# yanqinJiang/Animate3D

Measured on NVIDIA H100. Metric: MV-VDM denoise-steps/sec @ 4view x 16frame x 256^2, higher is better.
Workload: dtype fp16

## Files before the change

### animate3d_b200/csrc/a3d_gemm.cu

```cuda
#include <type_traits>

#include "a3d_common.cuh"
#include "a3d_host.cuh"
#include "a3d_wgmma.cuh"

namespace a3d {

struct GemmDev {
  int64_t M, N, K;
  int num_k_blocks;
  int tiles_m, tiles_n;
  int a_mode;
  int cpb;
  int conv_s;
  int tpi;
  int boh;
  int bimg;
  int tpr;
  int conv_pad;
  const float* bias;
  const float* rowbias;
  int64_t rb_ld, rb_div, rb_mod;
  float acc_scale;
  const __half* R1; int64_t ldr1; float r1_scale;
  const __half* R2; int64_t ldr2;
  void* C; int64_t ldc;
  int geglu, out_f32;
  int64_t perm_a, perm_b;
  long long* trace;
};

__device__ __forceinline__ float gelu_erf(float x) {
  float t;
  asm("rcp.approx.ftz.f32 %0, %1;" : "=f"(t) : "f"(fmaf(0.3275911f * 0.70710678118654752f, fabsf(x), 1.0f)));
  float poly = fmaf(1.061405429f, t, -1.453152027f);
  poly = fmaf(poly, t, 1.421413741f);
  poly = fmaf(poly, t, -0.284496736f);
  poly = fmaf(poly, t, 0.254829592f);
  const float xs = x * 0.84932180028801904f;
  const float e = ex2_approx(-xs * xs);
  const float erf_abs = fmaf(-(poly * t), e, 1.0f);
  const float h = 0.5f * x;
  return fmaf(fabsf(h), erf_abs, h);
}

__device__ __forceinline__ int64_t perm_row(int64_t m, int64_t a, int64_t b) {
  if (a == 0) return m;
  const int64_t ab = a * b;
  return (m / ab) * ab + (m % b) * a + (m / b) % a;
}

constexpr int kBM = 128;
constexpr int kBK = 64;
constexpr int kGemmThreads = 288;

template <int BN>
struct GemmCfg {
  static constexpr int kABytes = kBM * kBK * 2;
  static constexpr int kBBytes = BN * kBK * 2;
  static constexpr int kStageBytes = kABytes + kBBytes;
  static constexpr int kStages = (227 * 1024 - 1024 - 256) / kStageBytes > 6 ? 6 : (227 * 1024 - 1024 - 256) / kStageBytes;
  static constexpr int kSmemBytes = kStages * kStageBytes + 1024  + 256 ;
  static_assert(kSmemBytes <= 227 * 1024, "shared memory budget");
};

template <int BN>
__device__ __forceinline__ void wgmma_tile(float (&d)[BN / 2], uint64_t adesc, uint64_t bdesc, uint32_t acc) {
  if constexpr (BN == 256) wgmma_ss_n256<0>(d, adesc, bdesc, acc);
  else if constexpr (BN == 160) wgmma_ss_n160<0>(d, adesc, bdesc, acc);
  else wgmma_ss_n128<0>(d, adesc, bdesc, acc);
}

enum { kEpiPlain = 0, kEpiRes = 1, kEpiGeglu = 2, kEpiF32 = 3 };

template <int BN, int EPI>
struct EpiChunk {
  static constexpr int G = BN == 256 ? 1 + (EPI == kEpiGeglu) : 2;
  static constexpr bool kAhead = BN != 256;
  float bias[G][2];
  float rb[2][G][2];
  uint32_t r1[2][G], r2[2][G];
};

template <int EPI, int G>
__device__ __forceinline__ constexpr int epi_group(int c, int s) {
  if constexpr (EPI != kEpiGeglu) {
    return c * G + s;
  } else {
    const int o = c * (G / 2) + s % (G / 2);
    return (o / 4) * 8 + o % 4 + (s >= G / 2 ? 4 : 0);
  }
}

__device__ __forceinline__ void prefetch_l2(const void* a) { asm volatile("prefetch.global.L2 [%0];" ::"l"(a)); }

template <int BN, int EPI>
__global__ void __launch_bounds__(kGemmThreads, 1)
gemm_tc_kernel(const GemmDev p, const __grid_constant__ CUtensorMap mapA, const __grid_constant__ CUtensorMap mapB) {
  static_assert(EPI != kEpiGeglu || BN % 64 == 0, "GEGLU pairs a value with its gate inside 64-column blocks");
  static_assert((BN / 8) % EpiChunk<BN, EPI>::G == 0, "the tile's column groups split into whole chunks");
  using Cfg = GemmCfg<BN>;
  constexpr int kStages = Cfg::kStages;
  extern __shared__ uint8_t smem_raw[];
  uint8_t* smem = reinterpret_cast<uint8_t*>((reinterpret_cast<uintptr_t>(smem_raw) + 1023) & ~uintptr_t(1023));
  uint8_t* smem_a = smem;
  uint8_t* smem_b = smem + kStages * Cfg::kABytes;
  uint64_t* full_bar = reinterpret_cast<uint64_t*>(smem + kStages * Cfg::kStageBytes);
  uint64_t* empty_bar = full_bar + kStages;

  const int warp = threadIdx.x >> 5;
  const int lane = threadIdx.x & 31;
  const int num_tiles = p.tiles_m * p.tiles_n;

  if (warp == 8 && lane == 0) {
    tma_prefetch_desc(&mapA);
    tma_prefetch_desc(&mapB);
    for (int i = 0; i < kStages; ++i) {
      mbar_init(&full_bar[i], 1);
      mbar_init(&empty_bar[i], 8);
    }
    mbar_fence_init();
  }
  __syncthreads();

  if (warp == 8) {
    if (lane == 0) {
      int stage = 0;
      uint32_t phase = 0;
      for (int tile = blockIdx.x; tile < num_tiles; tile += gridDim.x) {
        const int mt = tile / p.tiles_n, nt = tile % p.tiles_n;
        int img0 = 0, oh0 = 0, ow0 = 0;
        if (p.a_mode == A3D_A_CONV3) {
          if (p.tpr > 1) { img0 = mt / p.tpi; oh0 = (mt % p.tpi) / p.tpr; ow0 = ((mt % p.tpi) % p.tpr) * kBM; }
          else if (p.tpi > 0) { img0 = mt / p.tpi; oh0 = (mt % p.tpi) * p.boh; }
          else { img0 = mt * p.bimg; oh0 = 0; }
        }
        for (int kb = 0; kb < p.num_k_blocks; ++kb) {
          mbar_wait(&empty_bar[stage], phase ^ 1);
          mbar_expect_tx(&full_bar[stage], Cfg::kStageBytes);
          if (p.a_mode == A3D_A_CONV3) {
            const int tap = kb / p.cpb, c0 = (kb % p.cpb) * kBK;
            const int ky = tap / 3, kx = tap % 3;
            tma_load_5d(smem_a + stage * Cfg::kABytes, &mapA, &full_bar[stage], c0, ow0 * p.conv_s + kx - p.conv_pad,
                        oh0 * p.conv_s + ky - p.conv_pad, img0, 0);
          } else {
            tma_load_5d(smem_a + stage * Cfg::kABytes, &mapA, &full_bar[stage], kb * kBK, mt * kBM, 0, 0, 0);
          }
          tma_load_5d(smem_b + stage * Cfg::kBBytes, &mapB, &full_bar[stage], kb * kBK, nt * BN, 0, 0, 0);
          if (++stage == kStages) { stage = 0; phase ^= 1; }
        }
      }
    }
    return;
  }

  const int wg = warp >> 2;
  const int g = lane >> 2, t = lane & 3;
  int stage = 0;
  uint32_t phase = 0;
  int tcount = 0;
  float acc[BN / 2];
  for (int tile = blockIdx.x; tile < num_tiles; tile += gridDim.x, ++tcount) {
    const int mt = tile / p.tiles_n, nt = tile % p.tiles_n;
    const bool tr = p.trace && blockIdx.x == 0 && threadIdx.x == 0 && tcount < 60;
    if (tr) p.trace[tcount * 16 + 0] = clock64();
    const int64_t col_base = (int64_t)nt * BN + 2 * t;
    int64_t row[2], orow[2];
#pragma unroll
    for (int h = 0; h < 2; ++h) {
      row[h] = (int64_t)mt * kBM + wg * 64 + (warp & 3) * 16 + g + 8 * h;
      orow[h] = (EPI == kEpiRes) ? perm_row(row[h], p.perm_a, p.perm_b) : row[h];
    }
    int prev_stage = -1;
    for (int kb = 0; kb < p.num_k_blocks; ++kb) {
      if constexpr (EPI == kEpiRes) {
        if (kb == (p.num_k_blocks > 2 ? p.num_k_blocks - 2 : 0)) {
          const int64_t ncols = p.N - (int64_t)nt * BN < BN ? p.N - (int64_t)nt * BN : BN;
          auto fetch = [&](const __half* a, bool ok) {
            const uintptr_t e = reinterpret_cast<uintptr_t>(a + ncols), l0 = reinterpret_cast<uintptr_t>(a) & ~uintptr_t(127);
#pragma unroll
            for (int i = 0; i < (2 * BN / 128 + 4) / 4; ++i) {
              const uintptr_t l = l0 + 128 * (t + 4 * i);
              if (ok && l < e) prefetch_l2(reinterpret_cast<const void*>(l));
            }
          };
#pragma unroll
          for (int h = 0; h < 2; ++h) {
            fetch(p.R1 + row[h] * p.ldr1 + (int64_t)nt * BN, p.R1 && row[h] < p.M);
            fetch(p.R2 + orow[h] * p.ldr2 + (int64_t)nt * BN, p.R2 && row[h] < p.M);
          }
        }
      }
      mbar_wait(&full_bar[stage], phase);
      const uint32_t a0 = smem_u32(smem_a + stage * Cfg::kABytes + wg * (64 * 128));
      const uint32_t b0 = smem_u32(smem_b + stage * Cfg::kBBytes);
      wgmma_fence();
#pragma unroll
      for (int k = 0; k < kBK / 16; ++k)
        wgmma_tile<BN>(acc, make_smem_desc_sw128(a0 + 32 * k, 16, 1024), make_smem_desc_sw128(b0 + 32 * k, 16, 1024),
                       (kb | k) ? 1u : 0u);
      wgmma_commit();
      wgmma_wait<1>();
      if (prev_stage >= 0 && lane == 0) mbar_arrive(&empty_bar[prev_stage]);
      prev_stage = stage;
      if (++stage == kStages) { stage = 0; phase ^= 1; }
    }

    using Chunk = EpiChunk<BN, EPI>;
    constexpr int G = Chunk::G;
    constexpr int kChunks = BN / 8 / G;
    const float* rb[2];
#pragma unroll
    for (int h = 0; h < 2; ++h) rb[h] = p.rowbias ? p.rowbias + ((row[h] / p.rb_div) % p.rb_mod) * p.rb_ld : nullptr;
    Chunk op;
    auto load_chunk = [&](int c) {
#pragma unroll
      for (int s = 0; s < G; ++s) {
        const int64_t n = col_base + 8 * epi_group<EPI, G>(c, s);
        const bool col_ok = n < p.N;
        op.bias[s][0] = (p.bias && col_ok) ? p.bias[n] : 0.f;
        op.bias[s][1] = (p.bias && col_ok) ? p.bias[n + 1] : 0.f;
#pragma unroll
        for (int h = 0; h < 2; ++h) {
          const bool ok = col_ok && row[h] < p.M;
          op.rb[h][s][0] = (rb[h] && ok) ? rb[h][n] : 0.f;
          op.rb[h][s][1] = (rb[h] && ok) ? rb[h][n + 1] : 0.f;
          if constexpr (EPI == kEpiRes) {
            op.r1[h][s] = (p.R1 && ok) ? *reinterpret_cast<const uint32_t*>(p.R1 + row[h] * p.ldr1 + n) : 0u;
            op.r2[h][s] = (p.R2 && ok) ? *reinterpret_cast<const uint32_t*>(p.R2 + orow[h] * p.ldr2 + n) : 0u;
          }
        }
      }
    };
    auto finish = [&](float v, int h, int s, int e) {
      if (p.bias) v += op.bias[s][e];
      if (rb[h]) v += op.rb[h][s][e];
      return v * p.acc_scale;
    };
    auto half2_float2 = [](uint32_t u) { return __half22float2(*reinterpret_cast<const __half2*>(&u)); };

    if constexpr (Chunk::kAhead) load_chunk(0);
    wgmma_wait<0>();
    reg_fence(acc);
    if (lane == 0) mbar_arrive(&empty_bar[prev_stage]);
    if (tr) p.trace[tcount * 16 + 1] = clock64();

#pragma unroll
    for (int c = 0; c < kChunks; ++c) {
      if constexpr (!Chunk::kAhead) load_chunk(c);
      if constexpr (EPI == kEpiGeglu) {
        uint32_t out[2][G / 2];
#pragma unroll
        for (int h = 0; h < 2; ++h)
#pragma unroll
          for (int s = 0; s < G / 2; ++s) {
            const int ju = epi_group<EPI, G>(c, s), jg = epi_group<EPI, G>(c, s + G / 2);
            const float u0 = finish(acc[4 * ju + 2 * h], h, s, 0), u1 = finish(acc[4 * ju + 2 * h + 1], h, s, 1);
            const float g0 = finish(acc[4 * jg + 2 * h], h, s + G / 2, 0), g1 = finish(acc[4 * jg + 2 * h + 1], h, s + G / 2, 1);
            out[h][s] = pack_f16x2(u0 * gelu_erf(g0), u1 * gelu_erf(g1));
          }
        if (Chunk::kAhead && c + 1 < kChunks) load_chunk(c + 1);
#pragma unroll
        for (int h = 0; h < 2; ++h) {
          if (row[h] >= p.M) continue;
          __half* crow = reinterpret_cast<__half*>(p.C) + row[h] * p.ldc;
#pragma unroll
          for (int s = 0; s < G / 2; ++s) {
            if (col_base + 8 * epi_group<EPI, G>(c, s) >= p.N) continue;
            const int o = c * (G / 2) + s;
            *reinterpret_cast<uint32_t*>(crow + (int64_t)nt * (BN / 2) + 8 * o + 2 * t) = out[h][s];
          }
        }
      } else if constexpr (EPI == kEpiF32) {
        float out[2][G][2];
#pragma unroll
        for (int h = 0; h < 2; ++h)
#pragma unroll
          for (int s = 0; s < G; ++s)
#pragma unroll
            for (int e = 0; e < 2; ++e) out[h][s][e] = finish(acc[4 * (c * G + s) + 2 * h + e], h, s, e);
        if (Chunk::kAhead && c + 1 < kChunks) load_chunk(c + 1);
#pragma unroll
        for (int h = 0; h < 2; ++h) {
          if (row[h] >= p.M) continue;
          float* crow = reinterpret_cast<float*>(p.C) + row[h] * p.ldc;
#pragma unroll
          for (int s = 0; s < G; ++s) {
            const int64_t n = col_base + 8 * (c * G + s);
            if (n >= p.N) continue;
            crow[n] = out[h][s][0];
            crow[n + 1] = out[h][s][1];
          }
        }
      } else {
        uint32_t out[2][G];
#pragma unroll
        for (int h = 0; h < 2; ++h)
#pragma unroll
          for (int s = 0; s < G; ++s) {
            const int j = c * G + s;
            float v0 = finish(acc[4 * j + 2 * h], h, s, 0), v1 = finish(acc[4 * j + 2 * h + 1], h, s, 1);
            if constexpr (EPI == kEpiRes) {
              if (p.R1) {
                const float2 f = half2_float2(op.r1[h][s]);
                v0 += p.r1_scale * f.x; v1 += p.r1_scale * f.y;
              }
              if (p.R2) {
                const float2 f = half2_float2(op.r2[h][s]);
                v0 += f.x; v1 += f.y;
              }
            }
            out[h][s] = pack_f16x2(v0, v1);
          }
        if (Chunk::kAhead && c + 1 < kChunks) load_chunk(c + 1);
#pragma unroll
        for (int h = 0; h < 2; ++h) {
          if (row[h] >= p.M) continue;
          __half* crow = reinterpret_cast<__half*>(p.C) + orow[h] * p.ldc;
#pragma unroll
          for (int s = 0; s < G; ++s) {
            const int64_t n = col_base + 8 * (c * G + s);
            if (n >= p.N) continue;
            *reinterpret_cast<uint32_t*>(crow + n) = out[h][s];
          }
        }
      }
    }
    if (tr) p.trace[tcount * 16 + 2] = clock64();
  }
}

struct SimtConv { int n, h, w, c, s, oh, ow, pad; };

__global__ void gemm_simt_kernel(const GemmDev p, const __half* __restrict__ A, int64_t lda, const __half* __restrict__ B,
                                 SimtConv cv) {
  const int64_t n_out = p.geglu ? p.N / 2 : p.N;
  const int64_t idx = (int64_t)blockIdx.x * blockDim.x + threadIdx.x;
  if (idx >= p.M * n_out) return;
  const int64_t m = idx / n_out;
  const int64_t j = idx % n_out;
  auto dot = [&](int64_t n) {
    float acc = 0.f;
    const __half* b = B + n * p.K;
    if (p.a_mode == A3D_A_PLAIN) {
      const __half* a = A + m * lda;
      for (int64_t k = 0; k < p.K; ++k) acc += __half2float(a[k]) * __half2float(b[k]);
    } else {
      const int img = (int)(m / (cv.oh * cv.ow));
      const int oy = (int)((m / cv.ow) % cv.oh), ox = (int)(m % cv.ow);
      for (int tap = 0; tap < 9; ++tap) {
        const int iy = oy * cv.s + tap / 3 - cv.pad, ix = ox * cv.s + tap % 3 - cv.pad;
        if (iy < 0 || iy >= cv.h || ix < 0 || ix >= cv.w) continue;
        const __half* a = A + (((int64_t)img * cv.h + iy) * cv.w + ix) * cv.c;
        const __half* bb = b + (int64_t)tap * cv.c;
        for (int c = 0; c < cv.c; ++c) acc += __half2float(a[c]) * __half2float(bb[c]);
      }
    }
    return acc;
  };
  const int64_t orow = perm_row(m, p.perm_a, p.perm_b);
  const float* rb = p.rowbias ? p.rowbias + ((m / p.rb_div) % p.rb_mod) * p.rb_ld : nullptr;
  auto finish = [&](int64_t n) {
    float v = dot(n);
    if (p.bias) v += p.bias[n];
    if (rb) v += rb[n];
    return v * p.acc_scale;
  };
  if (p.geglu) {
    const int64_t blk = j / 32, e = j % 32;
    const int64_t nu = blk * 64 + e, ng = nu + 32;
    const float u = finish(nu), g = finish(ng);
    reinterpret_cast<__half*>(p.C)[orow * p.ldc + j] = __float2half_rn(u * gelu_erf(g));
    return;
  }
  float v = finish(j);
  if (p.R1) v += p.r1_scale * __half2float(p.R1[m * p.ldr1 + j]);
  if (p.R2) v += __half2float(p.R2[orow * p.ldr2 + j]);
  if (p.out_f32) reinterpret_cast<float*>(p.C)[orow * p.ldc + j] = v;
  else reinterpret_cast<__half*>(p.C)[orow * p.ldc + j] = __float2half_rn(v);
}

template <int BN, int EPI>
static int launch_tc_epi(const GemmDev& dev, const CUtensorMap* mapA, const CUtensorMap* mapB, cudaStream_t st) {
  using Cfg = GemmCfg<BN>;
  static bool attr_set = false;
  if (!attr_set) {
    A3D_CUDA_CHECK(cudaFuncSetAttribute(gemm_tc_kernel<BN, EPI>, cudaFuncAttributeMaxDynamicSharedMemorySize, Cfg::kSmemBytes));
    attr_set = true;
  }
  const int tiles = dev.tiles_m * dev.tiles_n;
  const int grid = tiles < sm_count() ? tiles : sm_count();
  gemm_tc_kernel<BN, EPI><<<grid, kGemmThreads, Cfg::kSmemBytes, st>>>(dev, *mapA, *mapB);
  A3D_LAUNCH_CHECK();
  return A3D_OK;
}

template <int BN>
static int launch_tc(const GemmDev& dev, const CUtensorMap* mapA, const CUtensorMap* mapB, cudaStream_t st) {
  if (dev.out_f32) return launch_tc_epi<BN, kEpiF32>(dev, mapA, mapB, st);
  if (dev.geglu) {
    if constexpr (BN % 64 == 0) return launch_tc_epi<BN, kEpiGeglu>(dev, mapA, mapB, st);
    else return fail(A3D_EINVAL, "a3d_gemm: GEGLU needs a 128- or 256-column tile");
  }
  if (dev.R1 || dev.R2 || dev.perm_a) return launch_tc_epi<BN, kEpiRes>(dev, mapA, mapB, st);
  return launch_tc_epi<BN, kEpiPlain>(dev, mapA, mapB, st);
}

static long long* g_gemm_trace = nullptr;

}

extern "C" int a3d_debug_set_gemm_trace(void* device_buffer_1024_int64) {
  a3d::g_gemm_trace = reinterpret_cast<long long*>(device_buffer_1024_int64);
  return A3D_OK;
}

extern "C" int a3d_gemm(const a3d_gemm_args* a, void* stream) {
  using namespace a3d;
  cudaStream_t st = reinterpret_cast<cudaStream_t>(stream);
  if (!a || !a->A || !a->B || !a->C) return fail(A3D_EINVAL, "a3d_gemm: null operand");
  if (a->M <= 0 || a->N <= 0 || a->K <= 0) return fail(A3D_EINVAL, "a3d_gemm: empty problem M=%lld N=%lld K=%lld",
                                                        (long long)a->M, (long long)a->N, (long long)a->K);
  GemmDev d;
  memset(&d, 0, sizeof(d));
  d.M = a->M; d.N = a->N; d.K = a->K;
  d.a_mode = a->a_mode;
  d.bias = a->bias; d.rowbias = a->rowbias; d.rb_ld = a->rb_ld;
  d.rb_div = a->rb_div > 0 ? a->rb_div : 1; d.rb_mod = a->rb_mod > 0 ? a->rb_mod : (int64_t)1 << 40;
  d.acc_scale = a->acc_scale;
  d.R1 = reinterpret_cast<const __half*>(a->R1); d.ldr1 = a->ldr1; d.r1_scale = a->r1_scale;
  d.R2 = reinterpret_cast<const __half*>(a->R2); d.ldr2 = a->ldr2;
  d.C = a->C; d.ldc = a->ldc; d.geglu = a->geglu; d.out_f32 = a->out_f32;
  d.perm_a = a->perm_a; d.perm_b = a->perm_b;
  d.trace = g_gemm_trace;
  if (a->geglu && (a->out_f32 || a->R1 || a->R2 || a->perm_a || (a->N % 128)))
    return fail(A3D_EINVAL, "a3d_gemm: GEGLU epilogue takes bias / row-bias only, fp16 output, N %% 128 == 0");
  if (a->out_f32 && (a->R1 || a->R2 || a->perm_a))
    return fail(A3D_EINVAL, "a3d_gemm: fp32 output supports bias / row-bias only");

  SimtConv cv{0, 0, 0, 0, 1, 0, 0};
  if (a->a_mode == A3D_A_CONV3) {
    const int s = a->conv_stride;
    if (s != 1 && s != 2) return fail(A3D_EINVAL, "a3d_gemm: conv stride must be 1 or 2");
    if (a->conv_h % s || a->conv_w % s) return fail(A3D_EINVAL, "a3d_gemm: conv H/W must be multiples of the stride");
    cv = SimtConv{a->conv_n, a->conv_h, a->conv_w, a->conv_c, s, a->conv_h / s, a->conv_w / s, a->conv_nopad_lo ? 0 : 1};
    if (a->K != 9LL * a->conv_c || a->M != (int64_t)cv.n * cv.oh * cv.ow)
      return fail(A3D_EINVAL, "a3d_gemm: conv geometry does not match M/K");
    d.conv_s = s;
  } else if (a->a_mode != A3D_A_PLAIN) {
    return fail(A3D_EINVAL, "a3d_gemm: unknown a_mode %d", a->a_mode);
  }

  bool tc_ok = (a->K % kBK == 0) && (a->N % (a->geglu ? 16 : 8) == 0) && ((reinterpret_cast<uintptr_t>(a->A) & 15) == 0) &&
               ((reinterpret_cast<uintptr_t>(a->B) & 15) == 0) && (a->ldc % 16 == 0) &&
               ((reinterpret_cast<uintptr_t>(a->C) & 31) == 0);
  if (a->a_mode == A3D_A_PLAIN) tc_ok = tc_ok && (a->lda % 8 == 0) && a->lda >= a->K;
  int boh = 0, bimg = 1, tpi = 0, tpr = 1;
  if (a->a_mode == A3D_A_CONV3) {
    tc_ok = tc_ok && (cv.c % kBK == 0);
    const int opix = cv.oh * cv.ow;
    if (cv.ow > kBM) {
      tc_ok = tc_ok && (cv.ow % kBM == 0);
      boh = 1; tpr = cv.ow / kBM; tpi = cv.oh * tpr; bimg = 1;
    } else if (opix >= kBM) {
      tc_ok = tc_ok && (opix % kBM == 0) && (kBM % cv.ow == 0);
      boh = kBM / cv.ow; tpi = opix / kBM; bimg = 1;
    } else {
      tc_ok = tc_ok && (kBM % opix == 0);
      boh = cv.oh; tpi = 0; bimg = kBM / (opix > 0 ? opix : 1);
    }
    tc_ok = tc_ok && (tpr > 1 ? kBM : cv.ow) * cv.s <= 256 && boh * cv.s <= 256;
  }
  if (a->R1) tc_ok = tc_ok && (a->ldr1 % 16 == 0) && ((reinterpret_cast<uintptr_t>(a->R1) & 31) == 0);
  if (a->R2) tc_ok = tc_ok && (a->ldr2 % 16 == 0) && ((reinterpret_cast<uintptr_t>(a->R2) & 31) == 0);
  int impl = a->impl;
  if (impl == A3D_GEMM_AUTO) impl = tc_ok ? A3D_GEMM_TCGEN05 : A3D_GEMM_SIMT;
  if (impl == A3D_GEMM_TCGEN05 && !tc_ok)
    return fail(A3D_EINVAL, "a3d_gemm: shape/alignment not supported by the tensor-core path (M=%lld N=%lld K=%lld)",
                (long long)a->M, (long long)a->N, (long long)a->K);

  if (impl == A3D_GEMM_SIMT) {
    const int64_t n_out = a->geglu ? a->N / 2 : a->N;
    const int64_t total = a->M * n_out;
    const int threads = 128;
    const int64_t blocks = (total + threads - 1) / threads;
    gemm_simt_kernel<<<(unsigned)blocks, threads, 0, st>>>(d, reinterpret_cast<const __half*>(a->A), a->lda,
                                                           reinterpret_cast<const __half*>(a->B), cv);
    A3D_LAUNCH_CHECK();
    return A3D_OK;
  }

  int BN;
  if (a->geglu) BN = (a->N % 256 == 0) ? 256 : 128;
  else if (a->N % 256 == 0) BN = 256;
  else if (a->K <= 640 && a->N > 512 && (256 * ((a->N + 255) / 256) - a->N) * 8 <= a->N) {
    BN = 256;
  } else if (a->N % 160 == 0) BN = 160;
  else BN = 128;
  {
    static int force = -1;
    if (force < 0) { const char* e = getenv("A3D_GEMM_BN"); force = e ? atoi(e) : 0; }
    if (!a->geglu && (force == 128 || force == 160 || force == 256)) BN = force;
  }
  if (a->geglu && a->N % BN) return fail(A3D_EINVAL, "a3d_gemm: GEGLU needs N %% 128 == 0");
  d.num_k_blocks = (int)(a->K / kBK);
  d.tiles_m = (int)((a->M + kBM - 1) / kBM);
  d.tiles_n = (int)((a->N + BN - 1) / BN);
  d.cpb = a->a_mode == A3D_A_CONV3 ? cv.c / kBK : 0;
  d.tpi = tpi; d.boh = boh; d.bimg = bimg; d.tpr = tpr; d.conv_pad = cv.pad;
  const CUtensorMap *mapA = nullptr, *mapB = nullptr;
  {
    MapKey kb;
    const uint64_t dims[5] = {(uint64_t)a->K, (uint64_t)a->N, 1, 1, 1};
    const uint64_t str[4] = {(uint64_t)a->K, (uint64_t)a->K * a->N, (uint64_t)a->K * a->N, (uint64_t)a->K * a->N};
    const uint32_t box[5] = {kBK, (uint32_t)BN, 1, 1, 1};
    kb = make_key(a->B, dims, str, box);
    if (int r = get_tensor_map(kb, &mapB)) return r;
  }
  if (a->a_mode == A3D_A_PLAIN) {
    const uint64_t dims[5] = {(uint64_t)a->K, (uint64_t)a->M, 1, 1, 1};
    const uint64_t str[4] = {(uint64_t)a->lda, (uint64_t)a->lda * a->M, (uint64_t)a->lda * a->M, (uint64_t)a->lda * a->M};
    const uint32_t box[5] = {kBK, kBM, 1, 1, 1};
    MapKey ka = make_key(a->A, dims, str, box);
    if (int r = get_tensor_map(ka, &mapA)) return r;
  } else {
    const uint64_t img = (uint64_t)cv.h * cv.w * cv.c;
    const uint64_t dims[5] = {(uint64_t)cv.c, (uint64_t)cv.w, (uint64_t)cv.h, (uint64_t)cv.n, 1};
    const uint64_t str[4] = {(uint64_t)cv.c, (uint64_t)cv.w * cv.c, img, img * cv.n};
    const uint32_t box[5] = {kBK, (uint32_t)((tpr > 1 ? kBM : cv.ow) * cv.s), (uint32_t)(boh * cv.s), (uint32_t)bimg, 1};
    MapKey ka = make_key(a->A, dims, str, box);
    ka.estr[1] = cv.s; ka.estr[2] = cv.s;
    if (int r = get_tensor_map(ka, &mapA)) return r;
  }
  switch (BN) {
    case 256: return launch_tc<256>(d, mapA, mapB, st);
    case 160: return launch_tc<160>(d, mapA, mapB, st);
    default: return launch_tc<128>(d, mapA, mapB, st);
  }
}
```

Measured before the change: 5.606.

## Add B-panel-resident GEMM schedule with contiguous 64-row units per CTA

Adds a resident-B variant of the TMA/WGMMA GEMM for plain-epilogue, large-K, N%256 problems. Each CTA keeps a whole 128-column K-panel of B in shared memory and streams 64-row A units through a deep ring. The two warpgroups alternate units, handing off through named barriers, over a contiguous chunked range of tiles. The aim is to stop re-streaming B per tile and to let one warpgroup's epilogue overlap the other's MMA. The plain epilogue also switches to 16-byte stores via a quad shuffle transpose, at the cost of more complex synchronisation and a smaller N tile.

```diff
diff --git a/animate3d_b200/csrc/a3d_gemm.cu b/animate3d_b200/csrc/a3d_gemm.cu
--- a/animate3d_b200/csrc/a3d_gemm.cu
+++ b/animate3d_b200/csrc/a3d_gemm.cu
@@ -18,6 +18,8 @@
   int bimg;
   int tpr;
   int conv_pad;
+  int res_stages;
+  int res_chunks;
   const float* bias;
   const float* rowbias;
   int64_t rb_ld, rb_div, rb_mod;
@@ -64,6 +66,36 @@
   static_assert(kSmemBytes <= 227 * 1024, "shared memory budget");
 };
 
+constexpr int kUM = 64;
+constexpr int kUnitABytes = kUM * kBK * 2;
+struct ResidentCfg {
+  static constexpr int kBudget = 227 * 1024 - 1024  - 256 ;
+  static constexpr int kMinStages = 3, kMaxStages = 12;
+  static int stages(int64_t K, int BN) {
+    const int64_t s = (kBudget - K * BN * 2) / kUnitABytes;
+    return s < kMinStages ? 0 : s > kMaxStages ? kMaxStages : (int)s;
+  }
+  static int smem_bytes(int64_t K, int BN, int stages) { return (int)(K * BN * 2) + stages * kUnitABytes + 1024 + 256; }
+};
+
+struct Unit {
+  int m, nt;
+  int panel;
+};
+__device__ __forceinline__ int chunk_start(const GemmDev& p, int c) { return (int)((int64_t)c * p.tiles_m / p.res_chunks); }
+__device__ __forceinline__ Unit unit_at(const GemmDev& p, int64_t u) {
+  const int r = (int)(u / p.tiles_n);
+  int c = (int)((int64_t)r * p.res_chunks / p.tiles_m);
+  while (chunk_start(p, c + 1) <= r) ++c;
+  const int m0 = chunk_start(p, c), rows = chunk_start(p, c + 1) - m0;
+  const int w = (int)(u - (int64_t)p.tiles_n * m0);
+  return Unit{m0 + w % rows, w / rows, c * p.tiles_n + w / rows};
+}
+
+constexpr int kTurnBar = 1;
+__device__ __forceinline__ void named_bar_sync(int id, int n) { asm volatile("bar.sync %0, %1;" ::"r"(id), "r"(n) : "memory"); }
+__device__ __forceinline__ void named_bar_arrive(int id, int n) { asm volatile("bar.arrive %0, %1;" ::"r"(id), "r"(n) : "memory"); }
+
 template <int BN>
 __device__ __forceinline__ void wgmma_tile(float (&d)[BN / 2], uint64_t adesc, uint64_t bdesc, uint32_t acc) {
   if constexpr (BN == 256) wgmma_ss_n256<0>(d, adesc, bdesc, acc);
@@ -94,30 +126,55 @@
 
 __device__ __forceinline__ void prefetch_l2(const void* a) { asm volatile("prefetch.global.L2 [%0];" ::"l"(a)); }
 
-template <int BN, int EPI>
+__device__ __forceinline__ void quad_transpose(uint32_t (&w)[4], int t) {
+  const bool hi = t & 2, lo = t & 1;
+  const uint32_t k0 = hi ? w[2] : w[0], k1 = hi ? w[3] : w[1];
+  const uint32_t r0 = __shfl_xor_sync(0xffffffffu, hi ? w[0] : w[2], 2);
+  const uint32_t r1 = __shfl_xor_sync(0xffffffffu, hi ? w[1] : w[3], 2);
+  const uint32_t kk = lo ? k1 : k0, kr = lo ? r1 : r0;
+  const uint32_t xk = __shfl_xor_sync(0xffffffffu, lo ? k0 : k1, 1);
+  const uint32_t xr = __shfl_xor_sync(0xffffffffu, lo ? r0 : r1, 1);
+  const uint32_t a0 = lo ? xk : kk, a1 = lo ? kk : xk;
+  const uint32_t b0 = lo ? xr : kr, b1 = lo ? kr : xr;
+  w[0] = hi ? b0 : a0;
+  w[1] = hi ? b1 : a1;
+  w[2] = hi ? a0 : b0;
+  w[3] = hi ? a1 : b1;
+}
+
+template <int BN, int EPI, bool kResident>
 __global__ void __launch_bounds__(kGemmThreads, 1)
 gemm_tc_kernel(const GemmDev p, const __grid_constant__ CUtensorMap mapA, const __grid_constant__ CUtensorMap mapB) {
   static_assert(EPI != kEpiGeglu || BN % 64 == 0, "GEGLU pairs a value with its gate inside 64-column blocks");
   static_assert((BN / 8) % EpiChunk<BN, EPI>::G == 0, "the tile's column groups split into whole chunks");
   using Cfg = GemmCfg<BN>;
-  constexpr int kStages = Cfg::kStages;
+  const int stages = kResident ? p.res_stages : Cfg::kStages;
   extern __shared__ uint8_t smem_raw[];
   uint8_t* smem = reinterpret_cast<uint8_t*>((reinterpret_cast<uintptr_t>(smem_raw) + 1023) & ~uintptr_t(1023));
-  uint8_t* smem_a = smem;
-  uint8_t* smem_b = smem + kStages * Cfg::kABytes;
-  uint64_t* full_bar = reinterpret_cast<uint64_t*>(smem + kStages * Cfg::kStageBytes);
-  uint64_t* empty_bar = full_bar + kStages;
+  uint8_t* smem_a = kResident ? smem + p.num_k_blocks * Cfg::kBBytes : smem;
+  uint8_t* smem_b = kResident ? smem : smem + stages * Cfg::kABytes;
+  uint64_t* full_bar = reinterpret_cast<uint64_t*>(kResident ? smem_a + stages * kUnitABytes
+                                                             : smem + stages * Cfg::kStageBytes);
+  uint64_t* empty_bar = full_bar + stages;
+  uint64_t* panel_full = empty_bar + stages;
+  uint64_t* panel_empty = panel_full + 1;
 
   const int warp = threadIdx.x >> 5;
   const int lane = threadIdx.x & 31;
   const int num_tiles = p.tiles_m * p.tiles_n;
+  const int64_t u0 = (int64_t)num_tiles * blockIdx.x / gridDim.x;
+  const int n_run = (int)((int64_t)num_tiles * (blockIdx.x + 1) / gridDim.x - u0);
 
   if (warp == 8 && lane == 0) {
     tma_prefetch_desc(&mapA);
     tma_prefetch_desc(&mapB);
-    for (int i = 0; i < kStages; ++i) {
+    for (int i = 0; i < stages; ++i) {
       mbar_init(&full_bar[i], 1);
-      mbar_init(&empty_bar[i], 8);
+      mbar_init(&empty_bar[i], kResident ? 4 : 8);
+    }
+    if (kResident) {
+      mbar_init(panel_full, 1);
+      mbar_init(panel_empty, 8);
     }
     mbar_fence_init();
   }
@@ -127,27 +184,47 @@
     if (lane == 0) {
       int stage = 0;
       uint32_t phase = 0;
-      for (int tile = blockIdx.x; tile < num_tiles; tile += gridDim.x) {
-        const int mt = tile / p.tiles_n, nt = tile % p.tiles_n;
-        int img0 = 0, oh0 = 0, ow0 = 0;
-        if (p.a_mode == A3D_A_CONV3) {
-          if (p.tpr > 1) { img0 = mt / p.tpi; oh0 = (mt % p.tpi) / p.tpr; ow0 = ((mt % p.tpi) % p.tpr) * kBM; }
-          else if (p.tpi > 0) { img0 = mt / p.tpi; oh0 = (mt % p.tpi) * p.boh; }
-          else { img0 = mt * p.bimg; oh0 = 0; }
+      if constexpr (kResident) {
+        const int panel0 = unit_at(p, u0).panel;
+        for (int j = 0; j < n_run; ++j) {
+          const Unit u = unit_at(p, u0 + j);
+          const int s = u.panel - panel0;
+          if (j == 0 || s != unit_at(p, u0 + j - 1).panel - panel0) {
+            if (s > 0) mbar_wait(panel_empty, (s - 1) & 1);
+            mbar_expect_tx(panel_full, p.num_k_blocks * Cfg::kBBytes);
+            for (int kb = 0; kb < p.num_k_blocks; ++kb)
+              tma_load_5d(smem_b + kb * Cfg::kBBytes, &mapB, panel_full, kb * kBK, u.nt * BN, 0, 0, 0);
+          }
+          for (int kb = 0; kb < p.num_k_blocks; ++kb) {
+            mbar_wait(&empty_bar[stage], phase ^ 1);
+            mbar_expect_tx(&full_bar[stage], kUnitABytes);
+            tma_load_5d(smem_a + stage * kUnitABytes, &mapA, &full_bar[stage], kb * kBK, u.m * kUM, 0, 0, 0);
+            if (++stage == stages) { stage = 0; phase ^= 1; }
+          }
         }
-        for (int kb = 0; kb < p.num_k_blocks; ++kb) {
-          mbar_wait(&empty_bar[stage], phase ^ 1);
-          mbar_expect_tx(&full_bar[stage], Cfg::kStageBytes);
+      } else {
+        for (int tile = blockIdx.x; tile < num_tiles; tile += gridDim.x) {
+          const int mt = tile / p.tiles_n, nt = tile % p.tiles_n;
+          int img0 = 0, oh0 = 0, ow0 = 0;
           if (p.a_mode == A3D_A_CONV3) {
-            const int tap = kb / p.cpb, c0 = (kb % p.cpb) * kBK;
-            const int ky = tap / 3, kx = tap % 3;
-            tma_load_5d(smem_a + stage * Cfg::kABytes, &mapA, &full_bar[stage], c0, ow0 * p.conv_s + kx - p.conv_pad,
-                        oh0 * p.conv_s + ky - p.conv_pad, img0, 0);
-          } else {
-            tma_load_5d(smem_a + stage * Cfg::kABytes, &mapA, &full_bar[stage], kb * kBK, mt * kBM, 0, 0, 0);
-          }
-          tma_load_5d(smem_b + stage * Cfg::kBBytes, &mapB, &full_bar[stage], kb * kBK, nt * BN, 0, 0, 0);
-          if (++stage == kStages) { stage = 0; phase ^= 1; }
+            if (p.tpr > 1) { img0 = mt / p.tpi; oh0 = (mt % p.tpi) / p.tpr; ow0 = ((mt % p.tpi) % p.tpr) * kBM; }
+            else if (p.tpi > 0) { img0 = mt / p.tpi; oh0 = (mt % p.tpi) * p.boh; }
+            else { img0 = mt * p.bimg; oh0 = 0; }
+          }
+          for (int kb = 0; kb < p.num_k_blocks; ++kb) {
+            mbar_wait(&empty_bar[stage], phase ^ 1);
+            mbar_expect_tx(&full_bar[stage], Cfg::kStageBytes);
+            if (p.a_mode == A3D_A_CONV3) {
+              const int tap = kb / p.cpb, c0 = (kb % p.cpb) * kBK;
+              const int ky = tap / 3, kx = tap % 3;
+              tma_load_5d(smem_a + stage * Cfg::kABytes, &mapA, &full_bar[stage], c0, ow0 * p.conv_s + kx - p.conv_pad,
+                          oh0 * p.conv_s + ky - p.conv_pad, img0, 0);
+            } else {
+              tma_load_5d(smem_a + stage * Cfg::kABytes, &mapA, &full_bar[stage], kb * kBK, mt * kBM, 0, 0, 0);
+            }
+            tma_load_5d(smem_b + stage * Cfg::kBBytes, &mapB, &full_bar[stage], kb * kBK, nt * BN, 0, 0, 0);
+            if (++stage == stages) { stage = 0; phase ^= 1; }
+          }
         }
       }
     }
@@ -158,17 +235,54 @@
   const int g = lane >> 2, t = lane & 3;
   int stage = 0;
   uint32_t phase = 0;
-  int tcount = 0;
   float acc[BN / 2];
-  for (int tile = blockIdx.x; tile < num_tiles; tile += gridDim.x, ++tcount) {
-    const int mt = tile / p.tiles_n, nt = tile % p.tiles_n;
-    const bool tr = p.trace && blockIdx.x == 0 && threadIdx.x == 0 && tcount < 60;
-    if (tr) p.trace[tcount * 16 + 0] = clock64();
+  int panel0 = 0, panel = -1;
+  bool held = false;
+  if constexpr (kResident) {
+    panel0 = unit_at(p, u0).panel;
+    if (wg == 1) named_bar_arrive(kTurnBar, 256);
+  }
+  auto release_panel = [&] {
+    if (held && lane == 0) mbar_arrive(panel_empty);
+    held = false;
+  };
+  auto enter_panel = [&](int s) {
+    while (panel < s) {
+      release_panel();
+      ++panel;
+      held = true;
+      mbar_wait(panel_full, panel & 1);
+    }
+  };
+  for (int tcount = 0;; ++tcount) {
+    int nt;
+    int64_t row0;
+    bool panel_done = false;
+    if constexpr (kResident) {
+      const int j = wg + 2 * tcount;
+      if (j >= n_run) break;
+      const Unit u = unit_at(p, u0 + j);
+      enter_panel(u.panel - panel0);
+      nt = u.nt;
+      row0 = (int64_t)u.m * kUM;
+      panel_done = j + 2 >= n_run || unit_at(p, u0 + j + 2).panel != u.panel;
+      const int pos = j * p.num_k_blocks;
+      stage = pos % stages;
+      phase = (pos / stages) & 1;
+      named_bar_sync(kTurnBar + wg, 256);
+    } else {
+      const int tile = blockIdx.x + tcount * gridDim.x;
+      if (tile >= num_tiles) break;
+      nt = tile % p.tiles_n;
+      row0 = (int64_t)(tile / p.tiles_n) * kBM + wg * 64;
+    }
+    const bool tr = p.trace && blockIdx.x == 0 && (threadIdx.x & 127) == 0 && (kResident || wg == 0) && tcount < 60;
+    if (tr) p.trace[tcount * 16 + 3 * wg + 0] = clock64();
     const int64_t col_base = (int64_t)nt * BN + 2 * t;
     int64_t row[2], orow[2];
 #pragma unroll
     for (int h = 0; h < 2; ++h) {
-      row[h] = (int64_t)mt * kBM + wg * 64 + (warp & 3) * 16 + g + 8 * h;
+      row[h] = row0 + (warp & 3) * 16 + g + 8 * h;
       orow[h] = (EPI == kEpiRes) ? perm_row(row[h], p.perm_a, p.perm_b) : row[h];
     }
     int prev_stage = -1;
@@ -192,8 +306,9 @@
         }
       }
       mbar_wait(&full_bar[stage], phase);
-      const uint32_t a0 = smem_u32(smem_a + stage * Cfg::kABytes + wg * (64 * 128));
-      const uint32_t b0 = smem_u32(smem_b + stage * Cfg::kBBytes);
+      const uint32_t a0 = kResident ? smem_u32(smem_a + stage * kUnitABytes)
+                                    : smem_u32(smem_a + stage * Cfg::kABytes + wg * (64 * 128));
+      const uint32_t b0 = smem_u32(smem_b + (kResident ? kb : stage) * Cfg::kBBytes);
       wgmma_fence();
 #pragma unroll
       for (int k = 0; k < kBK / 16; ++k)
@@ -203,8 +318,10 @@
       wgmma_wait<1>();
       if (prev_stage >= 0 && lane == 0) mbar_arrive(&empty_bar[prev_stage]);
       prev_stage = stage;
-      if (++stage == kStages) { stage = 0; phase ^= 1; }
-    }
+      if (++stage == stages) { stage = 0; phase ^= 1; }
+    }
+    if constexpr (kResident)
+      if (wg + 2 * tcount + 1 < n_run) named_bar_arrive(kTurnBar + (wg ^ 1), 256);
 
     using Chunk = EpiChunk<BN, EPI>;
     constexpr int G = Chunk::G;
@@ -238,12 +355,24 @@
       return v * p.acc_scale;
     };
     auto half2_float2 = [](uint32_t u) { return __half22float2(*reinterpret_cast<const __half2*>(&u)); };
+    uint32_t quad[2][4];
+    auto store_quad = [&](int64_t n, int64_t n_end) {
+#pragma unroll
+      for (int h = 0; h < 2; ++h) {
+        quad_transpose(quad[h], t);
+        if (row[h] < p.M && n < n_end)
+          *reinterpret_cast<uint4*>(reinterpret_cast<__half*>(p.C) + orow[h] * p.ldc + n) =
+              make_uint4(quad[h][0], quad[h][1], quad[h][2], quad[h][3]);
+      }
+    };
 
     if constexpr (Chunk::kAhead) load_chunk(0);
     wgmma_wait<0>();
     reg_fence(acc);
     if (lane == 0) mbar_arrive(&empty_bar[prev_stage]);
-    if (tr) p.trace[tcount * 16 + 1] = clock64();
+    if constexpr (kResident)
+      if (panel_done) release_panel();
+    if (tr) p.trace[tcount * 16 + 3 * wg + 1] = clock64();
 
 #pragma unroll
     for (int c = 0; c < kChunks; ++c) {
@@ -313,21 +442,32 @@
             out[h][s] = pack_f16x2(v0, v1);
           }
         if (Chunk::kAhead && c + 1 < kChunks) load_chunk(c + 1);
-#pragma unroll
-        for (int h = 0; h < 2; ++h) {
-          if (row[h] >= p.M) continue;
-          __half* crow = reinterpret_cast<__half*>(p.C) + orow[h] * p.ldc;
+        if constexpr (EPI == kEpiPlain) {
 #pragma unroll
           for (int s = 0; s < G; ++s) {
-            const int64_t n = col_base + 8 * (c * G + s);
-            if (n >= p.N) continue;
-            *reinterpret_cast<uint32_t*>(crow + n) = out[h][s];
+            const int j = c * G + s;
+            quad[0][j % 4] = out[0][s];
+            quad[1][j % 4] = out[1][s];
+            if (j % 4 == 3) store_quad((int64_t)nt * BN + 8 * (j - 3 + t), p.N);
+          }
+        } else {
+#pragma unroll
+          for (int h = 0; h < 2; ++h) {
+            if (row[h] >= p.M) continue;
+            __half* crow = reinterpret_cast<__half*>(p.C) + orow[h] * p.ldc;
+#pragma unroll
+            for (int s = 0; s < G; ++s) {
+              const int64_t n = col_base + 8 * (c * G + s);
+              if (n >= p.N) continue;
+              *reinterpret_cast<uint32_t*>(crow + n) = out[h][s];
+            }
           }
         }
       }
     }
-    if (tr) p.trace[tcount * 16 + 2] = clock64();
-  }
+    if (tr) p.trace[tcount * 16 + 3 * wg + 2] = clock64();
+  }
+  if constexpr (kResident) enter_panel(unit_at(p, u0 + n_run - 1).panel - panel0);
 }
 
 struct SimtConv { int n, h, w, c, s, oh, ow, pad; };
@@ -380,30 +520,38 @@
   else reinterpret_cast<__half*>(p.C)[orow * p.ldc + j] = __float2half_rn(v);
 }
 
-template <int BN, int EPI>
-static int launch_tc_epi(const GemmDev& dev, const CUtensorMap* mapA, const CUtensorMap* mapB, cudaStream_t st) {
-  using Cfg = GemmCfg<BN>;
+template <int BN, int EPI, bool kResident>
+static int launch_tc_epi(const GemmDev& dev, const CUtensorMap* mapA, const CUtensorMap* mapB, int grid, cudaStream_t st) {
+  const int smem = kResident ? ResidentCfg::smem_bytes(dev.K, BN, dev.res_stages) : GemmCfg<BN>::kSmemBytes;
   static bool attr_set = false;
   if (!attr_set) {
-    A3D_CUDA_CHECK(cudaFuncSetAttribute(gemm_tc_kernel<BN, EPI>, cudaFuncAttributeMaxDynamicSharedMemorySize, Cfg::kSmemBytes));
+    A3D_CUDA_CHECK(cudaFuncSetAttribute(gemm_tc_kernel<BN, EPI, kResident>, cudaFuncAttributeMaxDynamicSharedMemorySize,
+                                        kResident ? 227 * 1024 : GemmCfg<BN>::kSmemBytes));
     attr_set = true;
   }
+  gemm_tc_kernel<BN, EPI, kResident><<<grid, kGemmThreads, smem, st>>>(dev, *mapA, *mapB);
+  A3D_LAUNCH_CHECK();
+  return A3D_OK;
+}
+
+template <int BN, int EPI>
+static int launch_tc_sched(const GemmDev& dev, const CUtensorMap* mapA, const CUtensorMap* mapB, cudaStream_t st) {
   const int tiles = dev.tiles_m * dev.tiles_n;
   const int grid = tiles < sm_count() ? tiles : sm_count();
-  gemm_tc_kernel<BN, EPI><<<grid, kGemmThreads, Cfg::kSmemBytes, st>>>(dev, *mapA, *mapB);
-  A3D_LAUNCH_CHECK();
-  return A3D_OK;
+  if constexpr (EPI == kEpiPlain && BN == 128)
+    if (dev.res_stages) return launch_tc_epi<BN, EPI, true>(dev, mapA, mapB, grid, st);
+  return launch_tc_epi<BN, EPI, false>(dev, mapA, mapB, grid, st);
 }
 
 template <int BN>
 static int launch_tc(const GemmDev& dev, const CUtensorMap* mapA, const CUtensorMap* mapB, cudaStream_t st) {
-  if (dev.out_f32) return launch_tc_epi<BN, kEpiF32>(dev, mapA, mapB, st);
+  if (dev.out_f32) return launch_tc_sched<BN, kEpiF32>(dev, mapA, mapB, st);
   if (dev.geglu) {
-    if constexpr (BN % 64 == 0) return launch_tc_epi<BN, kEpiGeglu>(dev, mapA, mapB, st);
+    if constexpr (BN % 64 == 0) return launch_tc_sched<BN, kEpiGeglu>(dev, mapA, mapB, st);
     else return fail(A3D_EINVAL, "a3d_gemm: GEGLU needs a 128- or 256-column tile");
   }
-  if (dev.R1 || dev.R2 || dev.perm_a) return launch_tc_epi<BN, kEpiRes>(dev, mapA, mapB, st);
-  return launch_tc_epi<BN, kEpiPlain>(dev, mapA, mapB, st);
+  if (dev.R1 || dev.R2 || dev.perm_a) return launch_tc_sched<BN, kEpiRes>(dev, mapA, mapB, st);
+  return launch_tc_sched<BN, kEpiPlain>(dev, mapA, mapB, st);
 }
 
 static long long* g_gemm_trace = nullptr;
@@ -497,15 +645,24 @@
     BN = 256;
   } else if (a->N % 160 == 0) BN = 160;
   else BN = 128;
-  {
-    static int force = -1;
-    if (force < 0) { const char* e = getenv("A3D_GEMM_BN"); force = e ? atoi(e) : 0; }
-    if (!a->geglu && (force == 128 || force == 160 || force == 256)) BN = force;
-  }
+  static int force = -1;
+  if (force < 0) { const char* e = getenv("A3D_GEMM_BN"); force = e ? atoi(e) : 0; }
+  const bool forced = !a->geglu && (force == 128 || force == 160 || force == 256);
+  if (forced) BN = force;
+  const bool resident = a->a_mode == A3D_A_PLAIN && !forced && BN == 256 && a->K >= 640 && ResidentCfg::stages(a->K, 128) &&
+                        !a->geglu && !a->out_f32 && !a->R1 && !a->R2 && !a->perm_a;
+  if (resident) BN = 128;
+  d.res_stages = resident ? ResidentCfg::stages(a->K, BN) : 0;
+  const int bm = d.res_stages ? kUM : kBM;
   if (a->geglu && a->N % BN) return fail(A3D_EINVAL, "a3d_gemm: GEGLU needs N %% 128 == 0");
   d.num_k_blocks = (int)(a->K / kBK);
-  d.tiles_m = (int)((a->M + kBM - 1) / kBM);
+  d.tiles_m = (int)((a->M + bm - 1) / bm);
   d.tiles_n = (int)((a->N + BN - 1) / BN);
+  if (d.res_stages) {
+    const int64_t units = (int64_t)d.tiles_m * d.tiles_n;
+    const int grid = units < sm_count() ? (int)units : sm_count();
+    d.res_chunks = grid / d.tiles_n < 1 ? 1 : grid / d.tiles_n > d.tiles_m ? d.tiles_m : grid / d.tiles_n;
+  }
   d.cpb = a->a_mode == A3D_A_CONV3 ? cv.c / kBK : 0;
   d.tpi = tpi; d.boh = boh; d.bimg = bimg; d.tpr = tpr; d.conv_pad = cv.pad;
   const CUtensorMap *mapA = nullptr, *mapB = nullptr;
@@ -520,7 +677,7 @@
   if (a->a_mode == A3D_A_PLAIN) {
     const uint64_t dims[5] = {(uint64_t)a->K, (uint64_t)a->M, 1, 1, 1};
     const uint64_t str[4] = {(uint64_t)a->lda, (uint64_t)a->lda * a->M, (uint64_t)a->lda * a->M, (uint64_t)a->lda * a->M};
-    const uint32_t box[5] = {kBK, kBM, 1, 1, 1};
+    const uint32_t box[5] = {kBK, (uint32_t)bm, 1, 1, 1};
     MapKey ka = make_key(a->A, dims, str, box);
     if (int r = get_tensor_map(ka, &mapA)) return r;
   } else {
```

Measured after the change: 5.778 (median of 6 runs). 1.03x the previous value.
